# nmdl-mizo/lcaonet

Measured on NVIDIA B200. Metric: molecules/sec fwd+bwd (QM9-shape), higher is better.
Workload: dtype f32

## Files before the change

### lcaonet_b200/csrc/gemm_tc.cu

```cuda
#include "common.cuh"

namespace {

constexpr int kEpiWarps = 4;
constexpr int kBlockM = 128;
constexpr int kChunkK = 32;
constexpr uint32_t kSpinLimit = 1u << 28;

__device__ __forceinline__ uint32_t smem_u32(const void* p) { return (uint32_t)__cvta_generic_to_shared(p); }

__device__ __forceinline__ void mbar_init(uint64_t* bar, uint32_t count) {
  asm volatile("mbarrier.init.shared::cta.b64 [%0], %1;" ::"r"(smem_u32(bar)), "r"(count));
}
__device__ __forceinline__ void mbar_arrive(uint64_t* bar) {
  asm volatile("mbarrier.arrive.shared::cta.b64 _, [%0];" ::"r"(smem_u32(bar)) : "memory");
}
__device__ __forceinline__ void mbar_wait(uint64_t* bar, uint32_t parity) {
  uint32_t done = 0, spins = 0;
  const uint32_t addr = smem_u32(bar);
  while (!done) {
    asm volatile(
        "{\n\t.reg .pred p;\n\t"
        "mbarrier.try_wait.parity.shared::cta.b64 p, [%1], %2;\n\t"
        "selp.u32 %0, 1, 0, p;\n\t}"
// ... 325 lines not shown
                o[0] += p0.x; o[1] += p0.y; o[2] += p0.z; o[3] += p0.w; o[4] += p1.x; o[5] += p1.y; o[6] += p1.z; o[7] += p1.w;
              }
              if (g.pre) store8(g.pre + m * g.ldp + c0 + j, o, wide);
              if (g.act == LCAO_ACT_SILU) {
#pragma unroll
                for (int q = 0; q < 8; ++q) o[q] = silu_fast(o[q]);
              }
              if (g.G) {
                const float4 h0 = gq[j / 4], h1 = gq[j / 4 + 1];
                o[0] *= silu_grad_fast(h0.x); o[1] *= silu_grad_fast(h0.y); o[2] *= silu_grad_fast(h0.z); o[3] *= silu_grad_fast(h0.w);
                o[4] *= silu_grad_fast(h1.x); o[5] *= silu_grad_fast(h1.y); o[6] *= silu_grad_fast(h1.z); o[7] *= silu_grad_fast(h1.w);
              }
              store8(g.Y + m * g.ldy + c0 + j, o, wide);
            }
          }
        }
        if (g.G) {
#pragma unroll
          for (int q = 0; q < 8; ++q) gq[q] = gn[q];
        }
      }
      tc_fence_before();
      mbar_arrive(&tempty[acc]);
    }
  }
  tc_fence_before();
  __syncthreads();
  if (warp == 8) {
    tc_fence_after();
    tmem_dealloc(tmem_base, tmem_cols);
  }
}

constexpr int kTaThreads = 15 * 32;
constexpr int kTaStages = 4;
constexpr uint32_t kTaCol0 = 256;

__device__ __forceinline__ void umma_tf32_ts(uint32_t tmem_d, uint32_t tmem_a, uint64_t desc_b, uint32_t idesc, uint32_t accumulate) {
  asm volatile(
      "{\n\t.reg .pred p;\n\t"
      "setp.ne.b32 p, %4, 0;\n\t"
      "tcgen05.mma.cta_group::1.kind::tf32 [%0], [%1], %2, %3, p;\n\t}"
      ::"r"(tmem_d), "r"(tmem_a), "l"(desc_b), "r"(idesc), "r"(accumulate)
      : "memory");
}
__device__ __forceinline__ void tmem_st32(uint32_t taddr, const uint32_t (&r)[32]) {
  asm volatile(
      "tcgen05.st.sync.aligned.32x32b.x32.b32 [%0], "
      "{%1,%2,%3,%4,%5,%6,%7,%8,%9,%10,%11,%12,%13,%14,%15,%16,%17,%18,%19,%20,%21,%22,%23,%24,%25,%26,%27,%28,%29,%30,%31,%32};"
      ::"r"(taddr), "r"(r[0]), "r"(r[1]), "r"(r[2]), "r"(r[3]), "r"(r[4]), "r"(r[5]), "r"(r[6]), "r"(r[7]), "r"(r[8]), "r"(r[9]),
        "r"(r[10]), "r"(r[11]), "r"(r[12]), "r"(r[13]), "r"(r[14]), "r"(r[15]), "r"(r[16]), "r"(r[17]), "r"(r[18]), "r"(r[19]),
        "r"(r[20]), "r"(r[21]), "r"(r[22]), "r"(r[23]), "r"(r[24]), "r"(r[25]), "r"(r[26]), "r"(r[27]), "r"(r[28]), "r"(r[29]),
        "r"(r[30]), "r"(r[31])
      : "memory");
}
__device__ __forceinline__ void tmem_ld32_nw(uint32_t taddr, float (&v)[32]) {
  asm volatile(
      "tcgen05.ld.sync.aligned.32x32b.x32.b32 "
      "{%0,%1,%2,%3,%4,%5,%6,%7,%8,%9,%10,%11,%12,%13,%14,%15,%16,%17,%18,%19,%20,%21,%22,%23,%24,%25,%26,%27,%28,%29,%30,%31}, [%32];"
      : "=f"(v[0]), "=f"(v[1]), "=f"(v[2]), "=f"(v[3]), "=f"(v[4]), "=f"(v[5]), "=f"(v[6]), "=f"(v[7]), "=f"(v[8]),
        "=f"(v[9]), "=f"(v[10]), "=f"(v[11]), "=f"(v[12]), "=f"(v[13]), "=f"(v[14]), "=f"(v[15]), "=f"(v[16]),
        "=f"(v[17]), "=f"(v[18]), "=f"(v[19]), "=f"(v[20]), "=f"(v[21]), "=f"(v[22]), "=f"(v[23]), "=f"(v[24]),
        "=f"(v[25]), "=f"(v[26]), "=f"(v[27]), "=f"(v[28]), "=f"(v[29]), "=f"(v[30]), "=f"(v[31])
      : "r"(taddr)
      : "memory");
}
__device__ __forceinline__ void tmem_wait_ld() { asm volatile("tcgen05.wait::ld.sync.aligned;" ::: "memory"); }
__device__ __forceinline__ void tmem_wait_st() { asm volatile("tcgen05.wait::st.sync.aligned;" ::: "memory"); }

__global__ void __launch_bounds__(kTaThreads, 1) k_tc_rows_ta(const RowsArgs g) {
  constexpr int kLd = 2;
  extern __shared__ __align__(1024) uint8_t smem_raw[];
  pdl_trigger();
  const int warp = threadIdx.x >> 5, lane = threadIdx.x & 31;
  const uint32_t blockB = g.Nb * 128;
  const uint32_t halfB = (g.Kc / kChunkK) * blockB;
  const int R = g.stages;
  uint8_t* sB = smem_raw;
  uint8_t* sRaw = sB + 2 * halfB;
  uint64_t* bars = reinterpret_cast<uint64_t*>(sRaw + (size_t)R * kStageBytes);
  uint64_t* raw_full = bars;
  uint64_t* raw_empty = raw_full + R;
  uint64_t* a_full = raw_empty + R;
  uint64_t* a_empty = a_full + kTaStages;
  uint64_t* tfull = a_empty + kTaStages;
  uint64_t* tempty = tfull + 2;
  uint32_t* tmem_slot = reinterpret_cast<uint32_t*>(tempty + 2);
  const int64_t nblocks = (g.M + kBlockM - 1) / kBlockM;
  const int nchunk = g.Kc / kChunkK;
  constexpr uint32_t tmem_cols = 512;

  if (threadIdx.x == 0) {
    for (int s = 0; s < R; ++s) {
      mbar_init(&raw_full[s], kLd * 32);
      mbar_init(&raw_empty[s], 4 * 32);
    }
    for (int s = 0; s < kTaStages; ++s) {
      mbar_init(&a_full[s], 4 * 32);
      mbar_init(&a_empty[s], 1);
    }
    for (int a = 0; a < 2; ++a) {
      mbar_init(&tfull[a], 1);
      mbar_init(&tempty[a], 2 * kEpiWarps * 32);
    }
    fence_barrier_init();
  }
  if (warp == 8) tmem_alloc(tmem_slot, tmem_cols);
  tc_fence_before();
  __syncthreads();
  tc_fence_after();
  const uint32_t tmem_base = *tmem_slot;

  constexpr int kStageThreads = (4 + 4 + 1) * 32;
  constexpr int kWB = 8;
  if (warp < 9) {
    const int kq = g.Kc / 4, total = g.Nb * kq;
    for (int base = 0; base < total; base += kWB * kStageThreads) {
      float4 w[kWB];
      int n[kWB], kg[kWB];
#pragma unroll
      for (int u = 0; u < kWB; ++u) {
        const int idx = base + u * kStageThreads + (int)threadIdx.x;
        w[u] = make_float4(0.f, 0.f, 0.f, 0.f);
        n[u] = -1;
        if (idx < total) {
          if (!g.b_trans) {
            n[u] = idx / kq; kg[u] = idx - n[u] * kq;
            w[u] = ldg4(g.W + (int64_t)n[u] * g.ldw + kg[u] * 4);
          } else {
            kg[u] = idx / g.Nb; n[u] = idx - kg[u] * g.Nb;
            w[u] = make_float4(__ldg(g.W + (int64_t)(kg[u] * 4 + 0) * g.ldw + n[u]), __ldg(g.W + (int64_t)(kg[u] * 4 + 1) * g.ldw + n[u]),
                               __ldg(g.W + (int64_t)(kg[u] * 4 + 2) * g.ldw + n[u]), __ldg(g.W + (int64_t)(kg[u] * 4 + 3) * g.ldw + n[u]));
          }
        }
      }
#pragma unroll
      for (int u = 0; u < kWB; ++u) {
        if (n[u] >= 0) {
          float4 hi, lo;
          split4(w[u], hi, lo);
          const uint32_t off = (kg[u] >> 3) * blockB + sw128_off(n[u], kg[u] & 7);
          *reinterpret_cast<float4*>(sB + off) = hi;
          *reinterpret_cast<float4*>(sB + halfB + off) = lo;
        }
      }
    }
    fence_proxy_async();
    asm volatile("bar.sync 1, %0;" ::"n"(kStageThreads) : "memory");
  }
  pdl_wait();

  if (warp >= 9 && warp < 9 + kLd) {
    constexpr int kRowsPerLd = kBlockM / kLd;
    const int lw = warp - 9, row_in = lane >> 3, c = lane & 7;
    const uint32_t raw_base = smem_u32(sRaw);
    uint32_t it = 0;
    for (int64_t mb = blockIdx.x; mb < nblocks; mb += gridDim.x) {
      const int64_t mrow = mb * kBlockM + kRowsPerLd * lw + row_in;
      for (int kc = 0; kc < nchunk; ++kc, ++it) {
        const int s = it % R;
        mbar_wait(&raw_empty[s], ((it / R) & 1) ^ 1);
        const uint32_t dst = raw_base + s * kStageBytes;
        const float* src = g.A + mrow * g.lda + kc * kChunkK + c * 4;
#pragma unroll
        for (int j = 0; j < kRowsPerLd / 4; ++j) {
          const bool ok = mrow + 4 * j < g.M;
          cp_async16(dst + sw128_off(kRowsPerLd * lw + 4 * j + row_in, c), ok ? src + (int64_t)4 * j * g.lda : g.A, ok ? 16u : 0u);
        }
        cp_async_arrive(&raw_full[s]);
      }
    }
  } else if (warp >= 4 && warp < 8) {
    const int row = (warp & 3) * 32 + lane;
    const uint32_t lane_base = (uint32_t)((warp & 3) * 32) << 16;
    uint32_t it = 0;
    for (int64_t mb = blockIdx.x; mb < nblocks; mb += gridDim.x) {
      for (int kc = 0; kc < nchunk; ++kc, ++it) {
        const int s = it % R, ts = it % kTaStages;
        mbar_wait(&raw_full[s], (it / R) & 1);
        mbar_wait(&a_empty[ts], ((it / kTaStages) & 1) ^ 1);
        tc_fence_after();
        const uint8_t* pr = sRaw + (size_t)s * kStageBytes;
        uint32_t hi[32], lo[32];
#pragma unroll
        for (int c = 0; c < 8; ++c) {
          const float4 v = *reinterpret_cast<const float4*>(pr + sw128_off(row, c));
          float4 h, l;
          split4(v, h, l);
          hi[4 * c] = __float_as_uint(h.x); hi[4 * c + 1] = __float_as_uint(h.y); hi[4 * c + 2] = __float_as_uint(h.z); hi[4 * c + 3] = __float_as_uint(h.w);
          lo[4 * c] = __float_as_uint(l.x); lo[4 * c + 1] = __float_as_uint(l.y); lo[4 * c + 2] = __float_as_uint(l.z); lo[4 * c + 3] = __float_as_uint(l.w);
        }
        const uint32_t ta = tmem_base + lane_base + kTaCol0 + ts * 64;
        tmem_st32(ta, hi);
        tmem_st32(ta + 32, lo);
        mbar_arrive(&raw_empty[s]);
        tmem_wait_st();
        tc_fence_before();
        mbar_arrive(&a_full[ts]);
      }
    }
  } else if (warp == 8) {
    {
      const uint32_t idesc = make_idesc(kBlockM, g.Nb);
      const uint32_t bBase = smem_u32(sB);
      uint32_t it = 0, tile = 0;
      for (int64_t mb = blockIdx.x; mb < nblocks; mb += gridDim.x, ++tile) {
        const int acc = tile & 1;
        mbar_wait(&tempty[acc], ((tile >> 1) & 1) ^ 1);
        tc_fence_after();
        const uint32_t d = tmem_base + acc * g.Nb;
        for (int kc = 0; kc < nchunk; ++kc, ++it) {
          const int ts = it % kTaStages;
          mbar_wait(&a_full[ts], (it / kTaStages) & 1);
          tc_fence_after();
          const uint32_t a_hi = tmem_base + kTaCol0 + ts * 64, a_lo = a_hi + 32;
          const uint32_t b_hi = bBase + kc * blockB, b_lo = b_hi + halfB;
          const uint64_t dBh0 = make_desc_sw128(b_hi), dBl0 = make_desc_sw128(b_lo);
#pragma unroll
          for (int kk = 0; kk < kChunkK / 8; ++kk) {
            const uint64_t dBh = dBh0 + 2 * kk, dBl = dBl0 + 2 * kk;
            if (elect_one()) {
              umma_tf32_ts(d, a_hi + kk * 8, dBh, idesc, (kc | kk) != 0);
              umma_tf32_ts(d, a_lo + kk * 8, dBh, idesc, 1);
              umma_tf32_ts(d, a_hi + kk * 8, dBl, idesc, 1);
            }
          }
          if (elect_one()) umma_commit(&a_empty[ts]);
        }
        if (elect_one()) umma_commit(&tfull[acc]);
      }
    }
    __syncwarp();
  } else if (warp < 4 || warp >= 9 + kLd) {
    const bool wide = g.wide_store != 0;
    const int quad = warp & 3;
    const int c_begin = warp >= 9 + kLd ? 64 : 0, c_end = min(g.Nb, c_begin + 64);
    uint32_t tile = 0;
    for (int64_t mb = blockIdx.x; mb < nblocks; mb += gridDim.x, ++tile) {
      const int acc = tile & 1;
      const int64_t m = mb * kBlockM + quad * 32 + lane;
      mbar_wait(&tfull[acc], (tile >> 1) & 1);
      tc_fence_after();
      float v[2][32];
      const uint32_t t0 = tmem_base + ((uint32_t)(quad * 32) << 16) + acc * g.Nb;
      if (c_begin < c_end) tmem_ld32_nw(t0 + c_begin, v[0]);
      if (c_begin + 32 < c_end) tmem_ld32_nw(t0 + c_begin + 32, v[1]);
      tmem_wait_ld();
      tc_fence_before();
      mbar_arrive(&tempty[acc]);
      if (m < g.M) {
#pragma unroll
        for (int h = 0; h < 2; ++h) {
          const int c0 = c_begin + 32 * h;
          if (c0 < c_end) {
            const int nc = min(32, c_end - c0);
#pragma unroll
            for (int j = 0; j < 32; j += 8) {
              if (j < nc) {
                float* o = v[h] + j;
                if (g.bias) {
                  const float4 b0 = ldg4(g.bias + c0 + j), b1 = ldg4(g.bias + c0 + j + 4);
                  o[0] += b0.x; o[1] += b0.y; o[2] += b0.z; o[3] += b0.w; o[4] += b1.x; o[5] += b1.y; o[6] += b1.z; o[7] += b1.w;
                }
                if (g.accumulate) {
                  const float4 p0 = *reinterpret_cast<const float4*>(g.Y + m * g.ldy + c0 + j);
                  const float4 p1 = *reinterpret_cast<const float4*>(g.Y + m * g.ldy + c0 + j + 4);
                  o[0] += p0.x; o[1] += p0.y; o[2] += p0.z; o[3] += p0.w; o[4] += p1.x; o[5] += p1.y; o[6] += p1.z; o[7] += p1.w;
                }
                if (g.pre) store8(g.pre + m * g.ldp + c0 + j, o, wide);
                if (g.act == LCAO_ACT_SILU) {
#pragma unroll
                  for (int q = 0; q < 8; ++q) o[q] = silu_fast(o[q]);
                }
                if (g.G) {
                  const float4 h0 = ldg4(g.G + m * g.ldg + c0 + j), h1 = ldg4(g.G + m * g.ldg + c0 + j + 4);
                  o[0] *= silu_grad_fast(h0.x); o[1] *= silu_grad_fast(h0.y); o[2] *= silu_grad_fast(h0.z); o[3] *= silu_grad_fast(h0.w);
                  o[4] *= silu_grad_fast(h1.x); o[5] *= silu_grad_fast(h1.y); o[6] *= silu_grad_fast(h1.z); o[7] *= silu_grad_fast(h1.w);
                }
                store8(g.Y + m * g.ldy + c0 + j, o, wide);
              }
            }
          }
        }
      }
    }
  }
  tc_fence_before();
  __syncthreads();
  if (warp == 8) {
    tc_fence_after();
    tmem_dealloc(tmem_base, tmem_cols);
  }
}

struct WgradArgs {
  const float* dY; int64_t ldy;
  const float* X; int64_t ldx;
  float* dW; int64_t ldw;
  float* db;
  float* part;
  int64_t M; int Kx; int x3, raw_stages, op_stages;
};

__global__ void __launch_bounds__(kRowsThreads, 1) k_tc_wgrad(const WgradArgs g) {
  extern __shared__ __align__(1024) uint8_t smem_raw[];
  const int warp = threadIdx.x >> 5, lane = threadIdx.x & 31;
  const uint32_t rawA = kChunkK * 512, rawB = kChunkK * g.Kx * 4;
  const uint32_t opA = 128 * 128, opB = g.Kx * 128;
  const uint32_t op_stage = (g.x3 ? 2 : 1) * (opA + opB);
  const int Rr = g.raw_stages, S = g.op_stages;
  uint8_t* sOp = smem_raw;
  uint8_t* sRaw = sOp + (size_t)S * op_stage;
  uint64_t* bars = reinterpret_cast<uint64_t*>(sRaw + (size_t)Rr * (rawA + rawB));
  uint64_t* raw_full = bars;
  uint64_t* raw_empty = raw_full + Rr;
  uint64_t* op_full = raw_empty + Rr;
  uint64_t* op_empty = op_full + S;
  uint64_t* tfull = op_empty + S;
  uint64_t* tempty = tfull + 2;
  uint32_t* tmem_slot = reinterpret_cast<uint32_t*>(tempty + 2);
  constexpr int kFlush = 8;
  const uint32_t acc_cols = g.x3 ? 2 * g.Kx : g.Kx;
  const uint32_t need_cols = 2 * acc_cols;
  const uint32_t tmem_cols = need_cols <= 32 ? 32 : need_cols <= 64 ? 64 : need_cols <= 128 ? 128 : need_cols <= 256 ? 256 : 512;

  const int64_t nchunks = (g.M + kChunkK - 1) / kChunkK;
  const int64_t per = (nchunks + gridDim.x - 1) / gridDim.x;
  const int64_t c_beg = min(nchunks, (int64_t)blockIdx.x * per), c_end = min(nchunks, c_beg + per);

  if (threadIdx.x == 0) {
    for (int s = 0; s < Rr; ++s) {
      mbar_init(&raw_full[s], kLoadWarps * 32);
      mbar_init(&raw_empty[s], 4 * 32);
    }
    for (int s = 0; s < S; ++s) {
      mbar_init(&op_full[s], 4 * 32);
      mbar_init(&op_empty[s], 1);
    }
    for (int a = 0; a < 2; ++a) {
      mbar_init(&tfull[a], 1);
      mbar_init(&tempty[a], kEpiWarps * 32);
    }
    fence_barrier_init();
  }
  if (warp == 8) tmem_alloc(tmem_slot, tmem_cols);
  tc_fence_before();
  __syncthreads();
  tc_fence_after();
  const uint32_t tmem_base = *tmem_slot;
  pdl_trigger();
  pdl_wait();
  if (c_beg >= c_end) {
    for (int i = threadIdx.x; i < g.Kx * 128; i += kRowsThreads) g.part[(size_t)blockIdx.x * g.Kx * 128 + i] = 0.f;
    if (g.db && threadIdx.x < 128) g.part[(size_t)gridDim.x * g.Kx * 128 + (size_t)blockIdx.x * 128 + threadIdx.x] = 0.f;
    __syncthreads();
    if (warp == 8) tmem_dealloc(tmem_base, tmem_cols);
    return;
  }

  if (warp >= 9) {
    const int lw = warp - 9, r_in = lane >> 3, pl = lane & 7;
    const uint32_t raw_base = smem_u32(sRaw);
    const int pgB = g.Kx / 32;
    uint32_t it = 0;
    for (int64_t c = c_beg; c < c_end; ++c, ++it) {
      const int s = it % Rr;
      mbar_wait(&raw_empty[s], ((it / Rr) & 1) ^ 1);
      const uint32_t dA = raw_base + s * (rawA + rawB), dB = dA + rawA;
      const int64_t m0 = c * kChunkK;
#pragma unroll
      for (int j = 0; j < 8; ++j) {
        const int r = 8 * lw + (j & 1) * 4 + r_in, pg = j >> 1;
        const bool ok = m0 + r < g.M;
        cp_async16(dA + r * 512 + (((pg * 8 + pl) ^ (r >> 2)) << 4), ok ? g.dY + (m0 + r) * g.ldy + (pg * 8 + pl) * 4 : g.dY,
                   ok ? 16u : 0u);
      }
      for (int j = 0; j < 2 * pgB; ++j) {
        const int r = 8 * lw + (j & 1) * 4 + r_in, pg = j >> 1;
        const bool ok = m0 + r < g.M;
        cp_async16(dB + r * (g.Kx * 4) + (((pg * 8 + pl) ^ (r >> 2)) << 4), ok ? g.X + (m0 + r) * g.ldx + (pg * 8 + pl) * 4 : g.X,
                   ok ? 16u : 0u);
      }
      cp_async_arrive(&raw_full[s]);
    }
  } else if (warp >= 4 && warp < 8) {
    const int t = threadIdx.x - 128;
    const int kg = t & 7, g0 = t >> 3;
    const int ngB = g.Kx / 4;
    float4 colsum[2] = {make_float4(0.f, 0.f, 0.f, 0.f), make_float4(0.f, 0.f, 0.f, 0.f)};
    uint32_t it = 0;
    for (int64_t c = c_beg; c < c_end; ++c, ++it) {
      const int r = it % Rr, s = it % S;
      mbar_wait(&raw_full[r], (it / Rr) & 1);
      mbar_wait(&op_empty[s], ((it / S) & 1) ^ 1);
      const uint8_t* rA = sRaw + (size_t)r * (rawA + rawB);
      const uint8_t* rB = rA + rawA;
      uint8_t* oA = sOp + (size_t)s * op_stage;
      uint8_t* oB = oA + (g.x3 ? 2 : 1) * opA;
#pragma unroll
      for (int i = 0; i < 2; ++i) {
        const int ng = g0 + 16 * i;
        float4 v[4];
#pragma unroll
        for (int q = 0; q < 4; ++q) v[q] = *reinterpret_cast<const float4*>(rA + (4 * kg + q) * 512 + ((ng ^ kg) << 4));
#pragma unroll
        for (int q = 0; q < 4; ++q)
          colsum[i] = make_float4(colsum[i].x + v[q].x, colsum[i].y + v[q].y, colsum[i].z + v[q].z, colsum[i].w + v[q].w);
        const float4 col[4] = {make_float4(v[0].x, v[1].x, v[2].x, v[3].x), make_float4(v[0].y, v[1].y, v[2].y, v[3].y),
                               make_float4(v[0].z, v[1].z, v[2].z, v[3].z), make_float4(v[0].w, v[1].w, v[2].w, v[3].w)};
#pragma unroll
        for (int j = 0; j < 4; ++j) {
          float4 hi, lo;
          split4(col[j], hi, lo);
          const uint32_t off = sw128_off(4 * ng + j, kg);
          *reinterpret_cast<float4*>(oA + off) = hi;
          if (g.x3) *reinterpret_cast<float4*>(oA + opA + off) = lo;
        }
      }
      for (int ng = g0; ng < ngB; ng += 16) {
        float4 v[4];
#pragma unroll
        for (int q = 0; q < 4; ++q)
          v[q] = *reinterpret_cast<const float4*>(rB + (4 * kg + q) * (g.Kx * 4) + ((ng ^ kg) << 4));
        const float4 col[4] = {make_float4(v[0].x, v[1].x, v[2].x, v[3].x), make_float4(v[0].y, v[1].y, v[2].y, v[3].y),
                               make_float4(v[0].z, v[1].z, v[2].z, v[3].z), make_float4(v[0].w, v[1].w, v[2].w, v[3].w)};
#pragma unroll
        for (int j = 0; j < 4; ++j) {
          float4 hi, lo;
          split4(col[j], hi, lo);
          const uint32_t off = sw128_off(4 * ng + j, kg);
          *reinterpret_cast<float4*>(oB + off) = hi;
          if (g.x3) *reinterpret_cast<float4*>(oB + opB + off) = lo;
        }
      }
      fence_proxy_async();
      mbar_arrive(&op_full[s]);
      mbar_arrive(&raw_empty[r]);
    }
    if (g.db) {
#pragma unroll
      for (int i = 0; i < 2; ++i) {
        float4 c = colsum[i];
#pragma unroll
        for (int o = 1; o < 8; o <<= 1) {
          c.x += __shfl_xor_sync(0xffffffffu, c.x, o); c.y += __shfl_xor_sync(0xffffffffu, c.y, o);
          c.z += __shfl_xor_sync(0xffffffffu, c.z, o); c.w += __shfl_xor_sync(0xffffffffu, c.w, o);
        }
        if (kg == 0)
          *reinterpret_cast<float4*>(g.part + (size_t)gridDim.x * g.Kx * 128 + (size_t)blockIdx.x * 128 + (g0 + 16 * i) * 4) = c;
      }
    }
  } else if (warp == 8) {
    {
      const uint32_t idesc = make_idesc(kBlockM, g.Kx);
      const uint32_t base = smem_u32(sOp);
      uint32_t it = 0, fl = 0;
      for (int64_t c = c_beg; c < c_end; ++fl) {
        const int acc = fl & 1;
        mbar_wait(&tempty[acc], ((fl >> 1) & 1) ^ 1);
        tc_fence_after();
        const uint32_t d = tmem_base + acc * acc_cols, dc = d + g.Kx;
        const int64_t c_stop = min(c_end, c + kFlush);
        for (int first = 1; c < c_stop; ++c, ++it) {
          const int s = it % S;
          mbar_wait(&op_full[s], (it / S) & 1);
          tc_fence_after();
          const uint32_t a_hi = base + s * op_stage, a_lo = a_hi + opA, b_hi = a_hi + (g.x3 ? 2 : 1) * opA, b_lo = b_hi + opB;
          const uint64_t dAh0 = make_desc_sw128(a_hi), dBh0 = make_desc_sw128(b_hi), dAl0 = make_desc_sw128(a_lo), dBl0 = make_desc_sw128(b_lo);
#pragma unroll
          for (int kk = 0; kk < kChunkK / 8; ++kk) {
            const uint64_t dAh = dAh0 + 2 * kk, dBh = dBh0 + 2 * kk, dAl = dAl0 + 2 * kk, dBl = dBl0 + 2 * kk;
            if (elect_one()) {
              umma_tf32(d, dAh, dBh, idesc, !first);
              if (g.x3) {
                umma_tf32(dc, dAl, dBh, idesc, !first);
                umma_tf32(dc, dAh, dBl, idesc, 1);
              }
            }
            first = 0;
          }
          if (elect_one()) umma_commit(&op_empty[s]);
        }
        if (elect_one()) umma_commit(&tfull[acc]);
      }
    }
    __syncwarp();
  } else {
    constexpr int kMaxCols = 128;
    float sum[kMaxCols];
#pragma unroll
    for (int j = 0; j < kMaxCols; ++j) sum[j] = 0.f;
    const int64_t n_flush = (c_end - c_beg + kFlush - 1) / kFlush;
    for (int64_t fl = 0; fl < n_flush; ++fl) {
      const int acc = fl & 1;
      mbar_wait(&tfull[acc], (fl >> 1) & 1);
      tc_fence_after();
      const uint32_t t0 = tmem_base + ((uint32_t)(warp * 32) << 16) + acc * acc_cols;
#pragma unroll
      for (int c0 = 0; c0 < kMaxCols; c0 += 32) {
        if (c0 < g.Kx) {
          float v[32];
          tmem_ld32(t0 + c0, v);
#pragma unroll
          for (int j = 0; j < 32; ++j) sum[c0 + j] += v[j];
          if (g.x3) {
            tmem_ld32(t0 + g.Kx + c0, v);
#pragma unroll
            for (int j = 0; j < 32; ++j) sum[c0 + j] += v[j];
          }
        }
      }
      tc_fence_before();
      mbar_arrive(&tempty[acc]);
    }
    const int n = warp * 32 + lane;
    float* pp = g.part + (size_t)blockIdx.x * g.Kx * 128 + n;
#pragma unroll
    for (int j = 0; j < kMaxCols; ++j)
      if (j < g.Kx) pp[(size_t)j * 128] = sum[j];
  }
  tc_fence_before();
  __syncthreads();
  if (warp == 8) {
    tc_fence_after();
    tmem_dealloc(tmem_base, tmem_cols);
  }
}

__global__ void __launch_bounds__(1024) k_wgrad_reduce(const float* __restrict__ part, int ncta, int Kx, float* __restrict__ dW,
                                                       int64_t ldw, float* __restrict__ db) {
  __shared__ float s_p[8][128];
  pdl_trigger();
  pdl_wait();
  const int j = blockIdx.x, n = threadIdx.x & 127, ty = threadIdx.x >> 7;
  const bool bias_row = j >= Kx;
  const float* src = bias_row ? part + (size_t)ncta * Kx * 128 + n : part + (size_t)j * 128 + n;
  const size_t stride = bias_row ? 128 : (size_t)Kx * 128;
  float acc = 0.f;
  for (int c = ty; c < ncta; c += 8) acc += src[(size_t)c * stride];
  s_p[ty][n] = acc;
  __syncthreads();
  if (ty == 0) {
    const float t = ((s_p[0][n] + s_p[1][n]) + (s_p[2][n] + s_p[3][n])) + ((s_p[4][n] + s_p[5][n]) + (s_p[6][n] + s_p[7][n]));
    if (bias_row) db[n] += t;
    else dW[(int64_t)n * ldw + j] += t;
  }
}

struct WgradDesc { const float* part; float* dW; float* db; int64_t ldw; int ncta, Kx; };
constexpr int kMaxWgradBatch = 32;
struct WgradBatch { WgradDesc d[kMaxWgradBatch]; };
__global__ void __launch_bounds__(1024) k_wgrad_reduce_batch(const WgradBatch b) {
  __shared__ float s_p[8][128];
  pdl_trigger();
  pdl_wait();
  const WgradDesc& g = b.d[blockIdx.y];
  const int j = blockIdx.x, n = threadIdx.x & 127, ty = threadIdx.x >> 7;
  if (j > g.Kx || (j == g.Kx && !g.db)) return;
  const bool bias_row = j >= g.Kx;
  const float* src = bias_row ? g.part + (size_t)g.ncta * g.Kx * 128 + n : g.part + (size_t)j * 128 + n;
  const size_t stride = bias_row ? 128 : (size_t)g.Kx * 128;
  float acc = 0.f;
  for (int c = ty; c < g.ncta; c += 8) acc += src[(size_t)c * stride];
  s_p[ty][n] = acc;
  __syncthreads();
  if (ty == 0) {
    const float t = ((s_p[0][n] + s_p[1][n]) + (s_p[2][n] + s_p[3][n])) + ((s_p[4][n] + s_p[5][n]) + (s_p[6][n] + s_p[7][n]));
    if (bias_row) g.db[n] += t;
    else g.dW[(int64_t)n * g.ldw + j] += t;
  }
}

constexpr size_t kMaxSmem = 227 * 1024;

int num_sms() {
  static int n = 0;
  if (n == 0) {
    int dev = 0;
    cudaGetDevice(&dev);
    cudaDeviceGetAttribute(&n, cudaDevAttrMultiProcessorCount, dev);
    if (n <= 0) n = 148;
  }
  return n;
}

inline bool al16(const void* p) { return (reinterpret_cast<uintptr_t>(p) & 15u) == 0; }

}

static size_t rows_smem(int Kc, int Nb, int stages, int lo_stages) {
  const size_t halfB = (size_t)(Kc / kChunkK) * Nb * 128;
  return 2 * halfB + (size_t)(stages + lo_stages) * kStageBytes + 512 + 1024;
}

bool lcao_tc_rows_ok(int64_t M, int Kc, int Nb, int64_t lda, int64_t ldy, const void* A, const void* Y) {
  return M >= 512 && Kc % 32 == 0 && Kc >= 32 && Nb % 16 == 0 && Nb >= 16 && Nb <= 128 && lda % 4 == 0 && ldy % 4 == 0 &&
         al16(A) && al16(Y) && rows_smem(Kc, Nb, 2, 2) <= kMaxSmem;
}

int lcao_tc_rows(const float* A, int64_t lda, const float* W, int64_t ldw, int b_trans, const float* bias, const float* G,
                 int64_t ldg, float* Y, int64_t ldy, float* pre, int64_t ldp, int64_t M, int Kc, int Nb, int act,
                 int accumulate, int x3, cudaStream_t st) {
  RowsArgs g{};
  g.A = A; g.lda = lda; g.W = W; g.ldw = ldw; g.bias = bias; g.G = G; g.ldg = ldg; g.Y = Y; g.ldy = ldy;
  g.pre = pre; g.ldp = ldp; g.M = M; g.Kc = Kc; g.Nb = Nb; g.b_trans = b_trans; g.act = act; g.accumulate = accumulate;
  g.x3 = x3;
  g.wide_store = ((reinterpret_cast<uintptr_t>(Y) | (uintptr_t)(ldy * 4)) & 31u) == 0 &&
                 (!pre || ((reinterpret_cast<uintptr_t>(pre) | (uintptr_t)(ldp * 4)) & 31u) == 0);
  int lo_stages = x3 ? 3 : 0;
  int stages = 8;
  while (stages > 2 && rows_smem(Kc, Nb, stages, lo_stages) > kMaxSmem) --stages;
  if (x3 && stages < 3 && lo_stages > 2) {
    lo_stages = 2;
    stages = 8;
    while (stages > 2 && rows_smem(Kc, Nb, stages, lo_stages) > kMaxSmem) --stages;
  }
  g.stages = stages;
  g.lo_stages = x3 ? lo_stages : 1;
  const size_t smem = rows_smem(Kc, Nb, stages, lo_stages);
  static bool attr_set = false;
  if (!attr_set) {
    LCAO_CUDA(cudaFuncSetAttribute(k_tc_rows<false>, cudaFuncAttributeMaxDynamicSharedMemorySize, (int)kMaxSmem));
    LCAO_CUDA(cudaFuncSetAttribute(k_tc_rows<true>, cudaFuncAttributeMaxDynamicSharedMemorySize, (int)kMaxSmem));
    attr_set = true;
  }
  const int64_t nblocks = (M + kBlockM - 1) / kBlockM;
  const unsigned grid = (unsigned)(nblocks < num_sms() ? nblocks : num_sms());
  const bool epi8 = nblocks <= num_sms();
  if (x3 && nblocks >= 2 * num_sms() && Nb <= 128 && Kc % kChunkK == 0 &&
      2 * (size_t)(Kc / kChunkK) * Nb * 128 + 3 * kStageBytes + 512 + 1024 <= kMaxSmem) {
    static bool ta_attr = false;
    if (!ta_attr) {
      LCAO_CUDA(cudaFuncSetAttribute(k_tc_rows_ta, cudaFuncAttributeMaxDynamicSharedMemorySize, (int)kMaxSmem));
      ta_attr = true;
    }
    const size_t halfB = (size_t)(Kc / kChunkK) * Nb * 128;
    int R = 8;
    while (R > 2 && 2 * halfB + (size_t)R * kStageBytes + 512 + 1024 > kMaxSmem) --R;
    g.stages = R;
    const size_t smem_ta = 2 * halfB + (size_t)R * kStageBytes + 512 + 1024;
    LCAO_CUDA(launch_pdl(k_tc_rows_ta, grid, kTaThreads, smem_ta, st, g));
    LCAO_LAUNCH_CHECK();
    return LCAO_OK;
  }
  if (epi8) LCAO_CUDA(launch_pdl(k_tc_rows<true>, grid, kRowsThreads + 128, smem, st, g));
  else LCAO_CUDA(launch_pdl(k_tc_rows<false>, grid, kRowsThreads, smem, st, g));
  LCAO_LAUNCH_CHECK();
  return LCAO_OK;
}

static size_t wgrad_smem(int Kx, int x3, int raw_stages, int op_stages) {
  const size_t raw = (size_t)kChunkK * (512 + Kx * 4), op = (size_t)(x3 ? 2 : 1) * (128 * 128 + Kx * 128);
  return (size_t)raw_stages * raw + (size_t)op_stages * op + 512 + 1024;
}

bool lcao_tc_wgrad_ok(int64_t M, int Kx, int64_t ldy, int64_t ldx, const void* dY, const void* X) {
  return M >= 512 && Kx % 32 == 0 && Kx >= 32 && Kx <= 128 && ldy % 4 == 0 && ldx % 4 == 0 && al16(dY) && al16(X) &&
         wgrad_smem(Kx, 1, 2, 2) <= kMaxSmem;
}

static unsigned wgrad_grid(int64_t M) {
  const int64_t want = (M + 127) / 128;
  return (unsigned)(want < 1 ? 1 : want < num_sms() ? want : num_sms());
}
int64_t lcao_tc_wgrad_scratch(int64_t M, int Kx) { return (int64_t)wgrad_grid(M) * ((int64_t)Kx * 128 + 128); }

int lcao_tc_wgrad(const float* dY, int64_t ldy, const float* X, int64_t ldx, float* dW, int64_t ldw, float* db, int64_t M,
                  int Kx, int x3, float* part, cudaStream_t st, int64_t* defer_desc) {
  WgradArgs g{};
  g.dY = dY; g.ldy = ldy; g.X = X; g.ldx = ldx; g.dW = dW; g.ldw = ldw; g.db = db; g.part = part;
  g.M = M; g.Kx = Kx; g.x3 = x3;
  g.op_stages = 2;
  int raw_stages = 6;
  while (raw_stages > 2 && wgrad_smem(Kx, x3, raw_stages, g.op_stages) > kMaxSmem) --raw_stages;
  g.raw_stages = raw_stages;
  static bool attr_set = false;
  if (!attr_set) {
    LCAO_CUDA(cudaFuncSetAttribute(k_tc_wgrad, cudaFuncAttributeMaxDynamicSharedMemorySize, (int)kMaxSmem));
    attr_set = true;
  }
  const unsigned grid = wgrad_grid(M);
  LCAO_CUDA(launch_pdl(k_tc_wgrad, grid, kRowsThreads, wgrad_smem(Kx, x3, raw_stages, g.op_stages), st, g));
  LCAO_LAUNCH_CHECK();
  if (defer_desc) {
    defer_desc[0] = (int64_t)(uintptr_t)part; defer_desc[1] = (int64_t)(uintptr_t)dW; defer_desc[2] = (int64_t)(uintptr_t)db;
    defer_desc[3] = ldw; defer_desc[4] = (int64_t)grid; defer_desc[5] = Kx;
    return LCAO_OK;
  }
  LCAO_CUDA(launch_pdl(k_wgrad_reduce, Kx + (db ? 1 : 0), 1024, 0, st, (const float*)part, (int)grid, Kx, dW, ldw, db));
  LCAO_LAUNCH_CHECK();
  return LCAO_OK;
}

int lcao_tc_wgrad_reduce_batch(const int64_t* desc, int n, cudaStream_t st) {
  for (int i0 = 0; i0 < n; i0 += kMaxWgradBatch) {
    WgradBatch b{};
    const int m = n - i0 < kMaxWgradBatch ? n - i0 : kMaxWgradBatch;
    int kmax = 0;
    for (int i = 0; i < m; ++i) {
      const int64_t* d = desc + 6 * (int64_t)(i0 + i);
      b.d[i].part = reinterpret_cast<const float*>((uintptr_t)d[0]);
      b.d[i].dW = reinterpret_cast<float*>((uintptr_t)d[1]);
      b.d[i].db = reinterpret_cast<float*>((uintptr_t)d[2]);
      b.d[i].ldw = d[3]; b.d[i].ncta = (int)d[4]; b.d[i].Kx = (int)d[5];
      kmax = b.d[i].Kx > kmax ? b.d[i].Kx : kmax;
    }
    LCAO_CUDA(launch_pdl(k_wgrad_reduce_batch, dim3((unsigned)(kmax + 1), (unsigned)m), 1024, 0, st, b));
    LCAO_LAUNCH_CHECK();
  }
  return LCAO_OK;
}
```

Measured before the change: 113,800.

## Stage wgrad A operand in tensor memory and split accumulator epilogue across warps

The weight-gradient kernel now writes the split hi/lo TF32 dY operand directly into tensor memory and issues TS-form MMAs, instead of transposing it into swizzled shared memory. It also accumulates all three x3 products into one accumulator rather than two. The epilogue is split across 8 warps, each summing half the columns with 16-wide TMEM loads, and the flush interval now depends on x3. The goal is to cut shared-memory traffic and transposition work and to shrink the smem footprint so more raw stages fit. The cost is a full 512-column TMEM allocation, extra barriers, and a different thread count.

```diff
diff --git a/lcaonet_b200/csrc/gemm_tc.cu b/lcaonet_b200/csrc/gemm_tc.cu
--- a/lcaonet_b200/csrc/gemm_tc.cu
+++ b/lcaonet_b200/csrc/gemm_tc.cu
@@ -651,27 +651,41 @@
   int64_t M; int Kx; int x3, raw_stages, op_stages;
 };
 
-__global__ void __launch_bounds__(kRowsThreads, 1) k_tc_wgrad(const WgradArgs g) {
+constexpr int kWgLd = 2;
+constexpr int kWgThreads = (17 + kWgLd) * 32;
+constexpr int kWgXf = 13 + kWgLd;
+__host__ __device__ constexpr int wgrad_flush(int x3) { return x3 ? 4 : 12; }
+
+__device__ __forceinline__ void tmem_ld16(uint32_t taddr, float (&v)[16]) {
+  asm volatile(
+      "tcgen05.ld.sync.aligned.32x32b.x16.b32 {%0,%1,%2,%3,%4,%5,%6,%7,%8,%9,%10,%11,%12,%13,%14,%15}, [%16];\n\t"
+      "tcgen05.wait::ld.sync.aligned;"
+      : "=f"(v[0]), "=f"(v[1]), "=f"(v[2]), "=f"(v[3]), "=f"(v[4]), "=f"(v[5]), "=f"(v[6]), "=f"(v[7]), "=f"(v[8]),
+        "=f"(v[9]), "=f"(v[10]), "=f"(v[11]), "=f"(v[12]), "=f"(v[13]), "=f"(v[14]), "=f"(v[15])
+      : "r"(taddr)
+      : "memory");
+}
+
+__global__ void __launch_bounds__(kWgThreads, 1) k_tc_wgrad(const WgradArgs g) {
   extern __shared__ __align__(1024) uint8_t smem_raw[];
   const int warp = threadIdx.x >> 5, lane = threadIdx.x & 31;
-  const uint32_t rawA = kChunkK * 512, rawB = kChunkK * g.Kx * 4;
-  const uint32_t opA = 128 * 128, opB = g.Kx * 128;
-  const uint32_t op_stage = (g.x3 ? 2 : 1) * (opA + opB);
+  const uint32_t rawA = kChunkK * 512, raw_stage = rawA + kChunkK * g.Kx * 4;
+  const uint32_t opB = g.Kx * 128;
+  const uint32_t op_stage = (g.x3 ? 2 : 1) * opB;
   const int Rr = g.raw_stages, S = g.op_stages;
   uint8_t* sOp = smem_raw;
   uint8_t* sRaw = sOp + (size_t)S * op_stage;
-  uint64_t* bars = reinterpret_cast<uint64_t*>(sRaw + (size_t)Rr * (rawA + rawB));
+  uint64_t* bars = reinterpret_cast<uint64_t*>(sRaw + (size_t)Rr * raw_stage);
   uint64_t* raw_full = bars;
   uint64_t* raw_empty = raw_full + Rr;
-  uint64_t* op_full = raw_empty + Rr;
-  uint64_t* op_empty = op_full + S;
-  uint64_t* tfull = op_empty + S;
+  uint64_t* a_full = raw_empty + Rr;
+  uint64_t* a_empty = a_full + kTaStages;
+  uint64_t* b_full = a_empty + kTaStages;
+  uint64_t* b_empty = b_full + S;
+  uint64_t* tfull = b_empty + S;
   uint64_t* tempty = tfull + 2;
   uint32_t* tmem_slot = reinterpret_cast<uint32_t*>(tempty + 2);
-  constexpr int kFlush = 8;
-  const uint32_t acc_cols = g.x3 ? 2 * g.Kx : g.Kx;
-  const uint32_t need_cols = 2 * acc_cols;
-  const uint32_t tmem_cols = need_cols <= 32 ? 32 : need_cols <= 64 ? 64 : need_cols <= 128 ? 128 : need_cols <= 256 ? 256 : 512;
+  constexpr uint32_t tmem_cols = 512;
 
   const int64_t nchunks = (g.M + kChunkK - 1) / kChunkK;
   const int64_t per = (nchunks + gridDim.x - 1) / gridDim.x;
@@ -679,16 +693,20 @@
 
   if (threadIdx.x == 0) {
     for (int s = 0; s < Rr; ++s) {
-      mbar_init(&raw_full[s], kLoadWarps * 32);
-      mbar_init(&raw_empty[s], 4 * 32);
+      mbar_init(&raw_full[s], kWgLd * 32);
+      mbar_init(&raw_empty[s], 2 * 4 * 32);
+    }
+    for (int s = 0; s < kTaStages; ++s) {
+      mbar_init(&a_full[s], 4 * 32);
+      mbar_init(&a_empty[s], 1);
     }
     for (int s = 0; s < S; ++s) {
-      mbar_init(&op_full[s], 4 * 32);
-      mbar_init(&op_empty[s], 1);
+      mbar_init(&b_full[s], 4 * 32);
+      mbar_init(&b_empty[s], 1);
     }
     for (int a = 0; a < 2; ++a) {
       mbar_init(&tfull[a], 1);
-      mbar_init(&tempty[a], kEpiWarps * 32);
+      mbar_init(&tempty[a], 2 * kEpiWarps * 32);
     }
     fence_barrier_init();
   }
@@ -700,14 +718,15 @@
   pdl_trigger();
   pdl_wait();
   if (c_beg >= c_end) {
-    for (int i = threadIdx.x; i < g.Kx * 128; i += kRowsThreads) g.part[(size_t)blockIdx.x * g.Kx * 128 + i] = 0.f;
+    for (int i = threadIdx.x; i < g.Kx * 128; i += kWgThreads) g.part[(size_t)blockIdx.x * g.Kx * 128 + i] = 0.f;
     if (g.db && threadIdx.x < 128) g.part[(size_t)gridDim.x * g.Kx * 128 + (size_t)blockIdx.x * 128 + threadIdx.x] = 0.f;
     __syncthreads();
     if (warp == 8) tmem_dealloc(tmem_base, tmem_cols);
     return;
   }
 
-  if (warp >= 9) {
+  if (warp >= 9 && warp < 9 + kWgLd) {
+    constexpr int kRg = kChunkK / 4 / kWgLd;
     const int lw = warp - 9, r_in = lane >> 3, pl = lane & 7;
     const uint32_t raw_base = smem_u32(sRaw);
     const int pgB = g.Kx / 32;
@@ -715,17 +734,16 @@
     for (int64_t c = c_beg; c < c_end; ++c, ++it) {
       const int s = it % Rr;
       mbar_wait(&raw_empty[s], ((it / Rr) & 1) ^ 1);
-      const uint32_t dA = raw_base + s * (rawA + rawB), dB = dA + rawA;
+      const uint32_t dA = raw_base + s * raw_stage, dB = dA + rawA;
       const int64_t m0 = c * kChunkK;
 #pragma unroll
-      for (int j = 0; j < 8; ++j) {
-        const int r = 8 * lw + (j & 1) * 4 + r_in, pg = j >> 1;
+      for (int j = 0; j < 4 * kRg; ++j) {
+        const int r = 4 * kRg * lw + (j % kRg) * 4 + r_in, pg = j / kRg;
         const bool ok = m0 + r < g.M;
-        cp_async16(dA + r * 512 + (((pg * 8 + pl) ^ (r >> 2)) << 4), ok ? g.dY + (m0 + r) * g.ldy + (pg * 8 + pl) * 4 : g.dY,
-                   ok ? 16u : 0u);
-      }
-      for (int j = 0; j < 2 * pgB; ++j) {
-        const int r = 8 * lw + (j & 1) * 4 + r_in, pg = j >> 1;
+        cp_async16(dA + r * 512 + ((pg * 8 + pl) << 4), ok ? g.dY + (m0 + r) * g.ldy + (pg * 8 + pl) * 4 : g.dY, ok ? 16u : 0u);
+      }
+      for (int j = 0; j < kRg * pgB; ++j) {
+        const int r = 4 * kRg * lw + (j % kRg) * 4 + r_in, pg = j / kRg;
         const bool ok = m0 + r < g.M;
         cp_async16(dB + r * (g.Kx * 4) + (((pg * 8 + pl) ^ (r >> 2)) << 4), ok ? g.X + (m0 + r) * g.ldx + (pg * 8 + pl) * 4 : g.X,
                    ok ? 16u : 0u);
@@ -733,39 +751,45 @@
       cp_async_arrive(&raw_full[s]);
     }
   } else if (warp >= 4 && warp < 8) {
-    const int t = threadIdx.x - 128;
+    const int n = (warp & 3) * 32 + lane;
+    const uint32_t lane_base = (uint32_t)((warp & 3) * 32) << 16;
+    float colsum = 0.f;
+    uint32_t it = 0;
+    for (int64_t c = c_beg; c < c_end; ++c, ++it) {
+      const int r = it % Rr, ts = it % kTaStages;
+      mbar_wait(&raw_full[r], (it / Rr) & 1);
+      mbar_wait(&a_empty[ts], ((it / kTaStages) & 1) ^ 1);
+      tc_fence_after();
+      const float* col = reinterpret_cast<const float*>(sRaw + (size_t)r * raw_stage) + n;
+      uint32_t hi[32], lo[32];
+#pragma unroll
+      for (int k = 0; k < kChunkK; ++k) {
+        const float v = col[k * 128];
+        colsum += v;
+        const float h = tf32_hi(v);
+        hi[k] = __float_as_uint(h);
+        lo[k] = __float_as_uint(tf32_hi(v - h));
+      }
+      const uint32_t ta = tmem_base + lane_base + kTaCol0 + ts * 64;
+      tmem_st32(ta, hi);
+      if (g.x3) tmem_st32(ta + 32, lo);
+      mbar_arrive(&raw_empty[r]);
+      tmem_wait_st();
+      tc_fence_before();
+      mbar_arrive(&a_full[ts]);
+    }
+    if (g.db) g.part[(size_t)gridDim.x * g.Kx * 128 + (size_t)blockIdx.x * 128 + n] = colsum;
+  } else if (warp >= kWgXf) {
+    const int t = threadIdx.x - kWgXf * 32;
     const int kg = t & 7, g0 = t >> 3;
     const int ngB = g.Kx / 4;
-    float4 colsum[2] = {make_float4(0.f, 0.f, 0.f, 0.f), make_float4(0.f, 0.f, 0.f, 0.f)};
     uint32_t it = 0;
     for (int64_t c = c_beg; c < c_end; ++c, ++it) {
       const int r = it % Rr, s = it % S;
       mbar_wait(&raw_full[r], (it / Rr) & 1);
-      mbar_wait(&op_empty[s], ((it / S) & 1) ^ 1);
-      const uint8_t* rA = sRaw + (size_t)r * (rawA + rawB);
-      const uint8_t* rB = rA + rawA;
-      uint8_t* oA = sOp + (size_t)s * op_stage;
-      uint8_t* oB = oA + (g.x3 ? 2 : 1) * opA;
-#pragma unroll
-      for (int i = 0; i < 2; ++i) {
-        const int ng = g0 + 16 * i;
-        float4 v[4];
-#pragma unroll
-        for (int q = 0; q < 4; ++q) v[q] = *reinterpret_cast<const float4*>(rA + (4 * kg + q) * 512 + ((ng ^ kg) << 4));
-#pragma unroll
-        for (int q = 0; q < 4; ++q)
-          colsum[i] = make_float4(colsum[i].x + v[q].x, colsum[i].y + v[q].y, colsum[i].z + v[q].z, colsum[i].w + v[q].w);
-        const float4 col[4] = {make_float4(v[0].x, v[1].x, v[2].x, v[3].x), make_float4(v[0].y, v[1].y, v[2].y, v[3].y),
-                               make_float4(v[0].z, v[1].z, v[2].z, v[3].z), make_float4(v[0].w, v[1].w, v[2].w, v[3].w)};
-#pragma unroll
-        for (int j = 0; j < 4; ++j) {
-          float4 hi, lo;
-          split4(col[j], hi, lo);
-          const uint32_t off = sw128_off(4 * ng + j, kg);
-          *reinterpret_cast<float4*>(oA + off) = hi;
-          if (g.x3) *reinterpret_cast<float4*>(oA + opA + off) = lo;
-        }
-      }
+      mbar_wait(&b_empty[s], ((it / S) & 1) ^ 1);
+      const uint8_t* rB = sRaw + (size_t)r * raw_stage + rawA;
+      uint8_t* oB = sOp + (size_t)s * op_stage;
       for (int ng = g0; ng < ngB; ng += 16) {
         float4 v[4];
 #pragma unroll
@@ -783,21 +807,8 @@
         }
       }
       fence_proxy_async();
-      mbar_arrive(&op_full[s]);
+      mbar_arrive(&b_full[s]);
       mbar_arrive(&raw_empty[r]);
-    }
-    if (g.db) {
-#pragma unroll
-      for (int i = 0; i < 2; ++i) {
-        float4 c = colsum[i];
-#pragma unroll
-        for (int o = 1; o < 8; o <<= 1) {
-          c.x += __shfl_xor_sync(0xffffffffu, c.x, o); c.y += __shfl_xor_sync(0xffffffffu, c.y, o);
-          c.z += __shfl_xor_sync(0xffffffffu, c.z, o); c.w += __shfl_xor_sync(0xffffffffu, c.w, o);
-        }
-        if (kg == 0)
-          *reinterpret_cast<float4*>(g.part + (size_t)gridDim.x * g.Kx * 128 + (size_t)blockIdx.x * 128 + (g0 + 16 * i) * 4) = c;
-      }
     }
   } else if (warp == 8) {
     {
@@ -808,65 +819,68 @@
         const int acc = fl & 1;
         mbar_wait(&tempty[acc], ((fl >> 1) & 1) ^ 1);
         tc_fence_after();
-        const uint32_t d = tmem_base + acc * acc_cols, dc = d + g.Kx;
-        const int64_t c_stop = min(c_end, c + kFlush);
+        const uint32_t d = tmem_base + acc * g.Kx;
+        const int64_t c_stop = min(c_end, c + wgrad_flush(g.x3));
         for (int first = 1; c < c_stop; ++c, ++it) {
-          const int s = it % S;
-          mbar_wait(&op_full[s], (it / S) & 1);
+          const int ts = it % kTaStages, s = it % S;
+          mbar_wait(&a_full[ts], (it / kTaStages) & 1);
+          mbar_wait(&b_full[s], (it / S) & 1);
           tc_fence_after();
-          const uint32_t a_hi = base + s * op_stage, a_lo = a_hi + opA, b_hi = a_hi + (g.x3 ? 2 : 1) * opA, b_lo = b_hi + opB;
-          const uint64_t dAh0 = make_desc_sw128(a_hi), dBh0 = make_desc_sw128(b_hi), dAl0 = make_desc_sw128(a_lo), dBl0 = make_desc_sw128(b_lo);
+          const uint32_t a_hi = tmem_base + kTaCol0 + ts * 64, a_lo = a_hi + 32;
+          const uint32_t b_hi = base + s * op_stage, b_lo = b_hi + opB;
+          const uint64_t dBh0 = make_desc_sw128(b_hi), dBl0 = make_desc_sw128(b_lo);
 #pragma unroll
           for (int kk = 0; kk < kChunkK / 8; ++kk) {
-            const uint64_t dAh = dAh0 + 2 * kk, dBh = dBh0 + 2 * kk, dAl = dAl0 + 2 * kk, dBl = dBl0 + 2 * kk;
+            const uint64_t dBh = dBh0 + 2 * kk, dBl = dBl0 + 2 * kk;
             if (elect_one()) {
-              umma_tf32(d, dAh, dBh, idesc, !first);
+              umma_tf32_ts(d, a_hi + kk * 8, dBh, idesc, !first);
               if (g.x3) {
-                umma_tf32(dc, dAl, dBh, idesc, !first);
-                umma_tf32(dc, dAh, dBl, idesc, 1);
+                umma_tf32_ts(d, a_lo + kk * 8, dBh, idesc, 1);
+                umma_tf32_ts(d, a_hi + kk * 8, dBl, idesc, 1);
               }
             }
             first = 0;
           }
-          if (elect_one()) umma_commit(&op_empty[s]);
+          if (elect_one()) {
+            umma_commit(&a_empty[ts]);
+            umma_commit(&b_empty[s]);
+          }
         }
         if (elect_one()) umma_commit(&tfull[acc]);
       }
     }
     __syncwarp();
   } else {
-    constexpr int kMaxCols = 128;
-    float sum[kMaxCols];
-#pragma unroll
-    for (int j = 0; j < kMaxCols; ++j) sum[j] = 0.f;
-    const int64_t n_flush = (c_end - c_beg + kFlush - 1) / kFlush;
+    constexpr int kMaxHalf = 64;
+    const int quad = warp & 3, half = g.Kx / 2;
+    const int j0 = warp >= 9 + kWgLd ? half : 0;
+    float sum[kMaxHalf];
+#pragma unroll
+    for (int j = 0; j < kMaxHalf; ++j) sum[j] = 0.f;
+    const int flush = wgrad_flush(g.x3);
+    const int64_t n_flush = (c_end - c_beg + flush - 1) / flush;
     for (int64_t fl = 0; fl < n_flush; ++fl) {
       const int acc = fl & 1;
       mbar_wait(&tfull[acc], (fl >> 1) & 1);
       tc_fence_after();
-      const uint32_t t0 = tmem_base + ((uint32_t)(warp * 32) << 16) + acc * acc_cols;
-#pragma unroll
-      for (int c0 = 0; c0 < kMaxCols; c0 += 32) {
-        if (c0 < g.Kx) {
-          float v[32];
-          tmem_ld32(t0 + c0, v);
-#pragma unroll
-          for (int j = 0; j < 32; ++j) sum[c0 + j] += v[j];
-          if (g.x3) {
-            tmem_ld32(t0 + g.Kx + c0, v);
-#pragma unroll
-            for (int j = 0; j < 32; ++j) sum[c0 + j] += v[j];
-          }
+      const uint32_t t0 = tmem_base + ((uint32_t)(quad * 32) << 16) + acc * g.Kx + j0;
+#pragma unroll
+      for (int c0 = 0; c0 < kMaxHalf; c0 += 16) {
+        if (c0 < half) {
+          float v[16];
+          tmem_ld16(t0 + c0, v);
+#pragma unroll
+          for (int j = 0; j < 16; ++j) sum[c0 + j] += v[j];
         }
       }
       tc_fence_before();
       mbar_arrive(&tempty[acc]);
     }
-    const int n = warp * 32 + lane;
-    float* pp = g.part + (size_t)blockIdx.x * g.Kx * 128 + n;
-#pragma unroll
-    for (int j = 0; j < kMaxCols; ++j)
-      if (j < g.Kx) pp[(size_t)j * 128] = sum[j];
+    const int n = quad * 32 + lane;
+    float* pp = g.part + (size_t)blockIdx.x * g.Kx * 128 + (size_t)j0 * 128 + n;
+#pragma unroll
+    for (int j = 0; j < kMaxHalf; ++j)
+      if (j < half) pp[(size_t)j * 128] = sum[j];
   }
   tc_fence_before();
   __syncthreads();
@@ -999,7 +1013,7 @@
 }
 
 static size_t wgrad_smem(int Kx, int x3, int raw_stages, int op_stages) {
-  const size_t raw = (size_t)kChunkK * (512 + Kx * 4), op = (size_t)(x3 ? 2 : 1) * (128 * 128 + Kx * 128);
+  const size_t raw = (size_t)kChunkK * (512 + Kx * 4), op = (size_t)(x3 ? 2 : 1) * Kx * 128;
   return (size_t)raw_stages * raw + (size_t)op_stages * op + 512 + 1024;
 }
 
@@ -1029,7 +1043,7 @@
     attr_set = true;
   }
   const unsigned grid = wgrad_grid(M);
-  LCAO_CUDA(launch_pdl(k_tc_wgrad, grid, kRowsThreads, wgrad_smem(Kx, x3, raw_stages, g.op_stages), st, g));
+  LCAO_CUDA(launch_pdl(k_tc_wgrad, grid, kWgThreads, wgrad_smem(Kx, x3, raw_stages, g.op_stages), st, g));
   LCAO_LAUNCH_CHECK();
   if (defer_desc) {
     defer_desc[0] = (int64_t)(uintptr_t)part; defer_desc[1] = (int64_t)(uintptr_t)dW; defer_desc[2] = (int64_t)(uintptr_t)db;
```

Result: no change. 114,800 (median of 6 runs) (+0.8%).
